# rrwick/Badread

Hardware: NVIDIA H100
Metric: simulated Gbases/sec (higher is better)
Workload: dtype u8/int32 (+f64 identity estimate)

## Files before the change

badread_b200/csrc/bb_api.cu:

```cuda
#include <cuda_runtime.h>
#include <dlfcn.h>
#include <unistd.h>

#include <algorithm>
#include <atomic>
#include <cstdio>
#include <cstdlib>
#include <cstring>
#include <numeric>
#include <string>
#include <thread>
#include <vector>

#include "bb_kernels.cuh"
#include "bb_launch.h"

namespace {

struct DevBuf {
    void *p = nullptr;
    size_t cap = 0;
    bool borrowed = false;
    void borrow(const DevBuf &o) { release(); p = o.p; cap = o.cap; borrowed = true; }
    cudaError_t ensure(size_t bytes) {
// ... 59 lines not shown
    DevBuf d_red;
    cudaEvent_t ev_scan = nullptr;
    DevBuf d_read_index, d_seg_off, d_segs, d_lit, d_target, d_order, d_reads;
    int n_lane_reads = 0, n_long_reads = 0;
    std::vector<int> h_order;
    DevBuf d_kidx, d_frag, d_state, d_seq, d_ops, d_dcnt, d_qual, d_out_seq, d_out_qual, d_counter, d_fpeq, d_speq, d_fallback;
    int64_t fpeq_total = 0;

    int n_warps = 0;
    BBScratchPool pool{}, pool_lean{};
    DevBuf s_hist, s_hbuf, s_lr, s_stack, s_tbuf, s_peq, s_ltbuf, s_leafhist, s_lr_lean, s_wckpt, s_lanehist;
    DevBuf d_ctime, d_chlog, d_wres, d_wtasks, d_wfallback, d_active;
    DevBuf p_q, p_t, p_ops, p_dcnt, p_out, p_qual;
    int lane8_cols = 4096;
    int pair_ctas = 1;
    bool head_worker = true;
    bool is_head = false;
    bool lpt_order = true;
    int ring_t = 4;
    bool lowmem = false;
    bool use_quad = false;
    int grid_div_env = 0;
    int grid_div = 1;
    struct QueueBufs { DevBuf node[BBQ_NODE_CLASSES][2], leaf[2], count; } qbuf[2];


    cudaEvent_t ev[BB_N_STAGES + 1] = {};
    float stage_ms[BB_N_STAGES] = {};

    std::vector<bb_ctx *> kids;
    int n_split = 1;
    std::vector<std::vector<int32_t>> part;
    std::vector<int64_t> part_base;
    cudaEvent_t ev_t0 = nullptr, ev_t1 = nullptr;

    bool trace = false;
    struct Mark { const char *name; int stream; cudaEvent_t ev; };
    std::vector<Mark> marks;
    std::vector<cudaEvent_t> mark_pool;
    size_t mark_used = 0;
};

static void mark(bb_ctx *ctx, cudaStream_t st, const char *name) {
    if (!ctx->trace) return;
    if (ctx->mark_used == ctx->mark_pool.size()) {
        cudaEvent_t e;
        if (cudaEventCreate(&e) != cudaSuccess) return;
// ... 135 lines not shown
    cudaEventCreate(&ctx->ev_t1);
    return BB_OK;
}

extern "C" int bb_destroy(bb_ctx *ctx) {
    if (!ctx) return BB_OK;
    for (bb_ctx *kid : ctx->kids) bb_destroy(kid);
    ctx->kids.clear();
    cudaSetDevice(ctx->device);
    cudaStreamSynchronize(ctx->stream);
    if (ctx->ev_t0) cudaEventDestroy(ctx->ev_t0);
    if (ctx->ev_t1) cudaEventDestroy(ctx->ev_t1);
    DevBuf *bufs[] = {&ctx->ref, &ctx->em_k2r, &ctx->em_hentries, &ctx->em_rowoff, &ctx->em_cum, &ctx->em_flags, &ctx->em_slots,
                      &ctx->em_pool, &ctx->em_rowinfo, &ctx->qm_hkeys, &ctx->qm_hvals, &ctx->qm_lkeys, &ctx->qm_lpool, &ctx->qm_rowoff, &ctx->qm_scores, &ctx->qm_cum,
                      &ctx->d_read_index, &ctx->d_seg_off, &ctx->d_segs, &ctx->d_lit, &ctx->d_target, &ctx->d_order,
                      &ctx->d_reads, &ctx->d_kidx, &ctx->d_frag, &ctx->d_state, &ctx->d_seq, &ctx->d_ops, &ctx->d_dcnt,
                      &ctx->d_qual, &ctx->d_out_seq, &ctx->d_out_qual, &ctx->d_counter, &ctx->s_hist, &ctx->s_hbuf,
                      &ctx->s_lr, &ctx->s_stack, &ctx->s_tbuf, &ctx->s_peq, &ctx->s_ltbuf, &ctx->d_ctime, &ctx->d_chlog, &ctx->d_wres,
                      &ctx->d_wtasks, &ctx->d_wfallback, &ctx->d_active,
                      &ctx->d_fpeq, &ctx->d_speq, &ctx->d_fallback, &ctx->s_leafhist, &ctx->s_lr_lean, &ctx->s_wckpt, &ctx->s_lanehist, &ctx->d_scan, &ctx->d_red,
                      &ctx->p_q, &ctx->p_t, &ctx->p_ops, &ctx->p_dcnt, &ctx->p_out, &ctx->p_qual};
    for (auto &qb : ctx->qbuf) {
        for (auto &cl : qb.node) for (auto &d : cl) d.release();
        qb.leaf[0].release(); qb.leaf[1].release(); qb.count.release();
    }
    for (DevBuf *b : bufs) b->release();
    for (auto &ev : ctx->ev) if (ev) cudaEventDestroy(ev);
    cudaStreamDestroy(ctx->stream);
    if (ctx->stream2) cudaStreamDestroy(ctx->stream2);
    if (ctx->ev_fork) cudaEventDestroy(ctx->ev_fork);
    if (ctx->ev_join) cudaEventDestroy(ctx->ev_join);
    if (ctx->ev_scan) cudaEventDestroy(ctx->ev_scan);
    for (int p = 0; p < 2; p++) {
        if (ctx->ev_level[p]) cudaEventDestroy(ctx->ev_level[p]);
        for (int x = 0; x < 3; x++) {
            if (ctx->side[p][x]) cudaStreamDestroy(ctx->side[p][x]);
            if (ctx->ev_side[p][x]) cudaEventDestroy(ctx->ev_side[p][x]);
        }
    }
    if (ctx->h_info) cudaFreeHost(ctx->h_info);
    if (ctx->nccl_comm && nccl_destroy) nccl_destroy(ctx->nccl_comm);
    for (cudaEvent_t e : ctx->mark_pool) cudaEventDestroy(e);
    delete ctx;
    return BB_OK;
}

template <typename T>
// ... 235 lines not shown
    {
        const size_t lanes = (size_t)lane_ctas * 64;
        if (ctx->lowmem) BB_CUDA(ctx, ctx->s_leafhist.ensure(2 * lanes * BB_LEAF_MAX_TILES * BB_LEAF_CKPT_WORDS * sizeof(uint32_t)));
        else BB_CUDA(ctx, ctx->s_lanehist.ensure(2 * lanes * BB_LEAF_LANE_COLS * BB_LEAF_LW * sizeof(uint2)));
        BB_CUDA(ctx, ctx->s_ltbuf.ensure(2 * lanes * BB_WIN_MAX_COLS));
        if (ctx->lowmem) BB_CUDA(ctx, ctx->s_wckpt.ensure(2 * lanes * BB_WIN_MAX_TILES * BB_WIN_CKPT_WORDS(BB_WIN_LW) * sizeof(uint32_t)));
    }
    const int len_b = (int)std::min<double>((double)ctx->max_len * ctx->slack + 64.0, (double)(1 << 24));
    const int lr_floor = ctx->lr_cap > 0 ? ctx->lr_cap : 4096;
    int lr_need = lr_floor;
    for (int r = 0; r < n; r++) {
        const double len = (double)ctx->h_reads[(size_t)r].frag_len;
        const double worst = len * ctx->slack + 64.0;
        const double expect = ctx->lr_cap > 0 ? 0.0 : 3.0 * (1.0 - ctx->h_target[(size_t)r]) * len + 0.02 * len + 512.0;
        lr_need = std::max(lr_need, (int)std::min(worst, ctx->lr_worst ? worst : expect));
    }
    int rc = ensure_scratch(ctx, len_b, lr_need, len_b, lr_floor);
    if (rc) return rc;
    const int cap_node = (int)std::min<int64_t>(ctx->seq_cap / 256 + 4ll * n + 1024, 0x7ffffff0);
    for (int s = 0; s < 2; s++) {
        auto &qb = ctx->qbuf[s];
        for (int c = 0; c < BBQ_NODE_CLASSES; c++)
            for (int p = 0; p < 2; p++) BB_CUDA(ctx, qb.node[c][p].ensure((size_t)cap_node * sizeof(BBNode)));
        for (int w = 0; w < 2; w++) BB_CUDA(ctx, qb.leaf[w].ensure((size_t)cap_node * sizeof(BBNode)));
        BB_CUDA(ctx, qb.count.ensure(512 * sizeof(int)));
    }
    ctx->n_levels = std::max(1, std::min(48, level_bound(ctx->max_len, ctx->slack) + ctx->extra_levels));
    return BB_OK;
}

static int w_batch_upload(bb_ctx *ctx, int32_t n_reads, const uint64_t *read_index, const int32_t *seg_off,
                          const bb_segment *segs, const uint8_t *literal_pool, int64_t literal_len,
                          const double *target_identity) {
    if (!ctx) return BB_ERR_ARG;
    if (n_reads <= 0 || !read_index || !seg_off || !segs || !target_identity || literal_len < 0)
        return set_err(ctx, BB_ERR_ARG, "bb_batch_upload: bad arguments");
    if (!ctx->have_em || !ctx->have_qm) return set_err(ctx, BB_ERR_STATE, "upload the error and qscore models first");
    BB_CUDA(ctx, cudaSetDevice(ctx->device));
    const int k = ctx->em.k;
    ctx->h_reads.assign((size_t)n_reads, BBReadDev{});
    ctx->h_inlen.assign((size_t)n_reads, 0);
    ctx->h_target.assign(target_identity, target_identity + n_reads);
    int64_t off = 0, peq_off = 0, log_off = 0, wres_off = 0;
    int max_len = 0;
    for (int32_t r = 0; r < n_reads; r++) {
        int64_t len = 0;
        if (seg_off[r + 1] < seg_off[r]) return set_err(ctx, BB_ERR_ARG, "seg_off must be non-decreasing");
// ... 85 lines not shown
                                 ctx->s_lanehist.as<uint2>(), ctx->s_ltbuf.as<uint8_t>(), c + BBC_LANE8, fb2, c + BBC_FB2);
        mark(ctx, st, "window_lane8");
        bbl_window_warp(pgrid(ctx, 2), st, B, ctx->em, ctx->pool, fb2, c + BBC_FB2, ctx->seed, c + BBC_WARP);
        mark(ctx, st, "window_warp");
        bb_k_replay<<<(n + 3) / 4, 128, 0, st>>>(B, order, n, ctx->em.k, c + BBC_PENDING);
        mark(ctx, st, "replay");
        ctx->launches += 6;
    }
    return BB_OK;
}

static int enqueue_align_tasks(bb_ctx *ctx, const BBBatchDev &B) {
    cudaStream_t stream[2] = {ctx->stream, ctx->stream2};
    const int n = ctx->n_reads;
    const int cap_node = (int)std::min<int64_t>(ctx->seq_cap / 256 + 4ll * n + 1024, 0x7ffffff0);
    const int lane_ctas = ctx->sm_count * 4;
    const size_t hist_per_pipe = (size_t)lane_ctas * 64 * BB_LEAF_MAX_TILES * BB_LEAF_CKPT_WORDS;
    BBQueues Q[2];
    int *cnt[2];
    for (int s = 0; s < 2; s++) {
        auto &qb = ctx->qbuf[s];
        for (int c = 0; c < BBQ_NODE_CLASSES; c++)
            for (int p = 0; p < 2; p++) Q[s].node[c][p] = qb.node[c][p].as<BBNode>();
        for (int w = 0; w < 2; w++) Q[s].leaf[w] = qb.leaf[w].as<BBNode>();
        cnt[s] = qb.count.as<int>();
        Q[s].count = cnt[s]; Q[s].overflow = cnt[s] + BBQ_OVERFLOW; Q[s].cap_node = cap_node; Q[s].cap_leaf = cap_node;
        Q[s].lane8_cols = ctx->lane8_cols;
        BB_CUDA(ctx, cudaMemsetAsync(cnt[s], 0, 512 * sizeof(int), stream[0]));
    }
    bb_k_push_roots<<<(n + 255) / 256, 256, 0, stream[0]>>>(B, Q[0], Q[1], ctx->d_order.as<int>());
    ctx->launches++;
    BB_CUDA(ctx, cudaEventRecord(ctx->ev_fork, stream[0]));
    BB_CUDA(ctx, cudaStreamWaitEvent(stream[1], ctx->ev_fork, 0));
    int *cursor[2] = {cnt[0] + 16, cnt[1] + 16};
    const int warp_base[2] = {0, ctx->n_warps / 2};
    const int w4 = ctx->sm_count * 4 * BB_WARPS_PER_CTA, w2 = ctx->sm_count * 6 * BB_WARPS_PER_CTA;
    const int lean_base[2] = {0, w4 + 2 * w2};
    for (int level = 0; level < ctx->n_levels; level++) {
        const int p = (level & 1) | (level > 0 && ctx->lpt_order ? BBQ_BACKWARDS : 0);
        for (int s = 0; s < 2; s++) {
            cudaStream_t st = stream[s];
            BB_CUDA(ctx, cudaMemsetAsync(cnt[s] + BBQ_COUNT(0, (p & 1) ^ 1), 0, BBQ_NODE_CLASSES * sizeof(int), st));
            BB_CUDA(ctx, cudaEventRecord(ctx->ev_level[s], st));
            int n_side = 0;
            auto on_side = [&]() -> cudaStream_t {
                cudaStream_t x = ctx->side[s][n_side++];
                cudaStreamWaitEvent(x, ctx->ev_level[s], 0);
                mark(ctx, x, "fork");
                return x;
            };
// ... 7 lines not shown
            {
                cudaStream_t x = on_side();
                bbl_node_warp(2, std::min(pgrid(ctx, 3, "WARP2"), ctx->sm_count * 6), x, B, Q[s], ctx->pool_lean, p, cursor[s]++, lean_base[s] + w4);
                mark(ctx, x, "node_warp2");
                bbl_node_warp(1, std::min(pgrid(ctx, 3, "WARP1"), ctx->sm_count * 6), x, B, Q[s], ctx->pool_lean, p, cursor[s]++, lean_base[s] + w4 + w2);
                mark(ctx, x, "node_warp1");
                x = on_side();
                bbl_node_lane8(pgrid(ctx, 6, "LANE8"), x, B, Q[s], p, cursor[s]++);
                mark(ctx, x, "node_lane8");
            }
            bbl_node_warp(4, std::min(pgrid(ctx, 2, "WARP4"), ctx->sm_count * 4), st, B, Q[s], ctx->pool_lean, p, cursor[s]++, lean_base[s]);
            mark(ctx, st, "node_warp4");
            ctx->launches += 4;
            for (int x = 0; x < n_side; x++) {
                BB_CUDA(ctx, cudaEventRecord(ctx->ev_side[s][x], ctx->side[s][x]));
                BB_CUDA(ctx, cudaStreamWaitEvent(st, ctx->ev_side[s][x], 0));
            }
        }
    }
    for (int s = 0; s < 2; s++) {
        cudaStream_t st = stream[s];
        bbl_leaf_warp(ctx->sm_count, st, B, Q[s], ctx->pool, cursor[s]++, warp_base[s]);
        mark(ctx, st, "leaf_warp");
        if (ctx->lowmem)
            bbl_leaf_lane(std::min(pgrid(ctx, 3, "LEAF"), ctx->sm_count * 4), st, B, Q[s], ctx->s_leafhist.as<uint32_t>() + s * hist_per_pipe, cursor[s]++);
        else
            bbl_leaf_lane_hist(std::min(pgrid(ctx, 4, "LEAF"), ctx->sm_count * 4), st, B, Q[s],
                               ctx->s_lanehist.as<uint2>() + s * ((size_t)lane_ctas * 64 * BB_LEAF_LANE_COLS * BB_LEAF_LW), cursor[s]++);
        mark(ctx, st, "leaf_lane");
        ctx->launches += 2;
    }
    BB_CUDA(ctx, cudaEventRecord(ctx->ev_join, stream[1]));
    BB_CUDA(ctx, cudaStreamWaitEvent(stream[0], ctx->ev_join, 0));
    for (int s = 0; s < 2; s++)
        BB_CUDA(ctx, cudaMemcpyAsync(ctx->h_info->qcount[s], cnt[s], 32 * sizeof(int), cudaMemcpyDeviceToHost, stream[0]));
    return BB_OK;
}

static int w_enqueue(bb_ctx *ctx) {
    if (!ctx) return BB_ERR_ARG;
    if (!ctx->uploaded) return set_err(ctx, BB_ERR_STATE, "bb_batch_run: no batch uploaded");
    BB_CUDA(ctx, cudaSetDevice(ctx->device));
    cudaStream_t st = ctx->stream;
    const int n = ctx->n_reads;
    BBBatchDev B = batch_dev(ctx);
    ctx->finished = false;
    BB_CUDA(ctx, cudaMemcpyAsync(ctx->d_reads.p, ctx->h_reads.data(), (size_t)n * sizeof(BBReadDev), cudaMemcpyHostToDevice, st));
    BB_CUDA(ctx, cudaMemsetAsync(ctx->d_counter.p, 0, BB_N_COUNTERS * sizeof(int), st));
    ctx->marks.clear(); ctx->mark_used = 0;
    mark(ctx, st, "begin");
    BB_CUDA(ctx, cudaEventRecord(ctx->ev[0], st));
    if (ctx->em.type == 1 && ctx->em_hash.entries)
        bb_k_build_fragments<0, true><<<n, 256, 0, st>>>(B, ctx->ref.as<uint8_t>(), ctx->em.k, ctx->seed, nullptr, ctx->em_hash);
// ... 602 lines not shown
```

badread_b200/csrc/bb_lane.cuh:

```cuda
#pragma once
#include <cstdint>

#include "bb_align.cuh"

struct BBLaneProb {
    const uint4 *peq;
    int peq_bit0;
    const uint8_t *q;
    int n;
    const uint8_t *t;
    int m;
    int a, b;
    uint2 *hist;
};

__device__ __forceinline__ int bb_lane_words(int a, int b) { return ((a + b) >> 5) + 2; }

__device__ __forceinline__ void bb_lane_fetch(const BBLaneProb &P, int word, uint32_t &mA, uint32_t &mC, uint32_t &mG,
                                              uint32_t &mT) {
    mA = mC = mG = mT = 0u;
    const int R = word * 32;
    const int valid = P.n - R;
    if (valid <= 0) return;
    const int s = P.peq_bit0 + R;
// ... 113 lines not shown

#define BB_RING_BYTES(LW, T) (2 * (T) * (LW) * 64 * 8)

__device__ __forceinline__ void bb_cp_async8(uint2 *smem, const uint2 *gmem) {
#if defined(__CUDA_ARCH__)
    asm volatile("cp.async.ca.shared.global [%0], [%1], 8;" ::"r"((uint32_t)__cvta_generic_to_shared(smem)), "l"(gmem) : "memory");
#else
    *smem = *gmem;
#endif
}
__device__ __forceinline__ void bb_cp_async_commit() {
#if defined(__CUDA_ARCH__)
    asm volatile("cp.async.commit_group;" ::: "memory");
#endif
}
template <int N>
__device__ __forceinline__ void bb_cp_async_wait() {
#if defined(__CUDA_ARCH__)
    asm volatile("cp.async.wait_group %0;" ::"n"(N) : "memory");
#endif
}

template <int LW, int T>
__device__ __forceinline__ void bb_ring_tick(uint2 *ring, const uint2 *hist, int tj, int &staged_lo) {
    const bool fresh = staged_lo > tj;
    if (fresh) {
        const int lo1 = max(0, tj - T + 1);
        for (int col = tj; col >= lo1; col--) {
#pragma unroll
            for (int x = 0; x < LW; x++) bb_cp_async8(ring + ((col & (2 * T - 1)) * LW + x) * 64, hist + (long long)col * LW + x);
        }
        bb_cp_async_commit();
        staged_lo = lo1;
    }
    const int want_lo = max(0, tj - 2 * T + 1);
    for (int col = staged_lo - 1; col >= want_lo; col--) {
#pragma unroll
        for (int x = 0; x < LW; x++) bb_cp_async8(ring + ((col & (2 * T - 1)) * LW + x) * 64, hist + (long long)col * LW + x);
    }
    bb_cp_async_commit();
    if (want_lo < staged_lo) staged_lo = want_lo;
#if defined(__CUDA_ARCH__)
    {
        constexpr int LINES = (T * LW * 8 + 127) / 128 + 1;
        const long long e = ((long long)tj - 4 * T) * LW;
#pragma unroll
        for (int x = 0; x < 2 * LINES; x++)
            if (e + 16 * x >= 0 && (x < LINES || fresh)) asm volatile("prefetch.global.L2 [%0];" ::"l"(hist + e + 16 * x));
    }
#endif
    bb_cp_async_wait<1>();
}

template <int LW, int T>
__device__ __forceinline__ uint2 bb_ring_entry(const uint2 *ring, int col, int x) {
    return ring[((col & (2 * T - 1)) * LW + x) * 64];
}
```

badread_b200/csrc/bb_launch.h:

```cpp
#pragma once
#include <cuda_runtime.h>

#include "bb_kernels.cuh"

void bbl_mutate(int grid, cudaStream_t st, BBBatchDev B, BBErrorModelDev em, unsigned long long seed, int *work_counter,
                const int *order, int n_items, bool chain);
cudaError_t bbl_window_lane_init();
void bbl_window_lane4(int grid, cudaStream_t st, BBBatchDev B, BBErrorModelDev em, const BBWinTask *tasks, const int *n_tasks,
                      unsigned long long seed, uint32_t *ckpt_pool, uint8_t *tbuf_pool, int *cursor, BBWinTask *fallback,
                      int *fallback_count);
void bbl_window_lane8(int grid, cudaStream_t st, BBBatchDev B, BBErrorModelDev em, const BBWinTask *tasks, const int *n_tasks,
                      unsigned long long seed, uint32_t *ckpt_pool, uint8_t *tbuf_pool, int *cursor, BBWinTask *fallback,
                      int *fallback_count);
void bbl_window_lane_hist(int words, int ring_t, int grid, cudaStream_t st, BBBatchDev B, BBErrorModelDev em, const BBWinTask *tasks,
                          const int *n_tasks, unsigned long long seed, uint2 *hist_pool, uint8_t *tbuf_pool, int *cursor,
                          BBWinTask *fallback, int *fallback_count);
void bbl_window_warp(int grid, cudaStream_t st, BBBatchDev B, BBErrorModelDev em, BBScratchPool pool, const BBWinTask *tasks,
                     const int *n_tasks, unsigned long long seed, int *cursor);
void bbl_node_warp(int words, int grid, cudaStream_t st, BBBatchDev B, BBQueues Q, BBScratchPool pool, int parity, int *cursor,
                   int warp_base);
void bbl_node_lane8(int grid, cudaStream_t st, BBBatchDev B, BBQueues Q, int parity, int *cursor);
cudaError_t bbl_node_quad_init();
void bbl_node_quad(int grid, cudaStream_t st, BBBatchDev B, BBQueues Q, BBScratchPool pool, int parity, int *cursor,
                   int warp_base);
cudaError_t bbl_node_pair_init();
void bbl_node_pair(int grid, cudaStream_t st, BBBatchDev B, BBQueues Q, BBScratchPool pool, int parity, int *cursor,
                   int warp_base);
void bbl_leaf_warp(int grid, cudaStream_t st, BBBatchDev B, BBQueues Q, BBScratchPool pool, int *cursor, int warp_base);
void bbl_leaf_lane_hist(int grid, cudaStream_t st, BBBatchDev B, BBQueues Q, uint2 *hist_pool, int *cursor);
cudaError_t bbl_leaf_lane_init();
void bbl_leaf_lane(int grid, cudaStream_t st, BBBatchDev B, BBQueues Q, uint32_t *ckpt_pool, int *cursor);
void bbl_align_pair(cudaStream_t st, const uint8_t *q, int n, const uint8_t *t, int m, int k_upper, BBScratchPool pool,
                    uint8_t *ops, unsigned int *dcnt, int *out5);
```

badread_b200/csrc/bb_loop.cuh:

```cuda
#pragma once
#include <cstdint>

#include "bb_lane.cuh"

enum { BB_STOP_HORIZON = 0, BB_STOP_LIMIT = 1, BB_STOP_COUNT = 2, BB_STOP_NOLOOP = 3 };

#define BB_WIN_LW 8
#define BB_WIN_MAX_COLS 2048

struct BBWinTask { int r, a; };

#define BB_MUTP_THREADS (BB_WARPS_PER_CTA * 32 + 32)

template <int BB_TU_ = 0>
__global__ void __launch_bounds__(BB_MUTP_THREADS)
bb_k_mutate(BBBatchDev B, BBErrorModelDev em, unsigned long long seed, int *work_counter, const int *order,
                 int n_items) {
    constexpr int NE = BB_WARPS_PER_CTA * 32;
    __shared__ int s_kind[2][NE], s_pos[2][NE], s_rpos[2][NE];
    __shared__ uint32_t s_pay[2][NE];
    __shared__ int s_w, s_stop, s_cc;
    __shared__ long long s_n0;
    const int lane = threadIdx.x & 31;
    const int warp = threadIdx.x >> 5;
// ... 414 lines not shown
#endif
template <int LW, int T = BB_WIN_RING_T>
__global__ void __launch_bounds__(64, (LW <= 4 ? 8 : 4))
bb_k_window_lane_hist(BBBatchDev B, BBErrorModelDev em, const BBWinTask *tasks, const int *n_tasks_ptr, unsigned long long seed,
                 uint2 *hist_pool, uint8_t *tbuf_pool, int *cursor, BBWinTask *fallback, int *fallback_count) {
#ifdef BB_EMULATOR
    static uint2 s_ring[BB_RING_BYTES(LW, T) / 8];
#else
    extern __shared__ __align__(16) uint2 s_ring[];
#endif
    const int n_tasks = *n_tasks_ptr;
    const long long gl = (long long)blockIdx.x * blockDim.x + threadIdx.x;
    uint2 *const hist = hist_pool + gl * (long long)(BB_WIN_MAX_COLS * LW);
    uint8_t *const tbuf = tbuf_pool + gl * (long long)BB_WIN_MAX_COLS;
    uint2 *const ring = s_ring + threadIdx.x;
    BBLanePass<LW> S;
    BBProb P;
    BBWinTask tk = {0, 0};
    const uint8_t *frag = nullptr;
    const uint32_t *state = nullptr;
    const unsigned int *ctime = nullptr;
    int phase = 0;
    int qpos = 0, qn = 0, jx = 0, tm = 0, uw = 0, ti = 0, tj = 0, diags = 0, dels = 0, dist = 0, staged_lo = 0;
    unsigned int tmax = 0;
    for (;;) {
        if (phase == 0) {
            const int w = atomicAdd(cursor, 1);
            if (w >= n_tasks) phase = 4;
            else {
                tk = tasks[w];
                const BBReadDev *rd = &B.reads[tk.r];
                frag = B.frag + rd->frag_off; state = B.state + rd->frag_off; ctime = B.ctime + rd->frag_off;
                bb_window_of(rd->frag_len, seed, B.read_index[tk.r], tk.a, qpos, qn);
                tmax = (unsigned int)(BB_ALIGNMENT_INTERVAL * tk.a);
                jx = 0; tm = 0; uw = 0;
                phase = 1;
            }
        }
        if (__all_sync(BB_FULL, phase == 4)) break;
        for (int it = 0; it < 64; it++) {
            if (phase == 1) {
                unsigned int ct4[4];
                uint8_t fb4[4];
#pragma unroll
                for (int h = 0; h < 4; h++) {
                    const int j = min(jx + h, qn - 1);
// ... 6 lines not shown
                        if (ct4[h] == 0u || ct4[h] > tmax) { if (tm < BB_WIN_MAX_COLS) tbuf[tm] = fb4[h]; tm++; }
                        else {
                            const uint32_t st = state[qpos + jx];
                            const int sl = (int)(st & 0xff);
                            for (int c = 0; c < sl; c++) { if (tm < BB_WIN_MAX_COLS) tbuf[tm] = bb_slot_char(em, st, c); tm++; }
                            uw += sl < 1 ? 1 : sl;
                        }
                        jx++;
                    }
                }
                if (jx >= qn) {
                    const int diff = qn > tm ? qn - tm : tm - qn;
                    if (uw < diff) uw = diff;
                    const int mx = qn > tm ? qn : tm;
                    if (uw > mx) uw = mx;
                    bb_band(qn, tm, uw, P.a, P.b);
                    if (tm > BB_WIN_MAX_COLS || bb_lane_words(P.a, P.b) > LW || !bb_uses_traceback(qn, tm)) {
                        fallback[atomicAdd(fallback_count, 1)] = tk;
                        phase = 0;
                    } else {
                        const BBReadDev *rd = &B.reads[tk.r];
                        P.n = qn; P.peq = B.fpeq + rd->fpeq_off; P.q = frag + qpos; P.qs = 1;
                        P.peq_bit0 = qpos + BB_PEQ_BIT0; P.t = tbuf; P.ts = 1;
                        bb_lane_begin<LW>(S, P);
                        phase = 2;
                    }
                }
            }
        }
        for (int it = 0; it < 128; it++) {
            if (phase == 2) {
                bb_lane_step<LW, true>(S, P, hist + (long long)S.c * LW);
                if (S.c >= tm) {
                    dist = bb_lane_corner<LW>(S, qn);
                    ti = qn - 1; tj = tm - 1; diags = 0; dels = 0; staged_lo = tm; phase = 3;
                }
            }
        }
        for (int it = 0; it < 256; it++) {
            if (phase == 3) {
                if (ti >= 0 && tj >= 0) {
                    if ((it & (T - 1)) == 0) bb_ring_tick<LW, T>(ring, hist, tj, staged_lo);
                    int wt = (tj - P.a) >> 5; if (wt < 0) wt = 0;
                    const int x = (ti >> 5) - wt;
                    if (x < 0 || x >= LW) { atomicOr(&B.reads[tk.r].flags, 1); ti = -1; tj = -1; }
                    else {
                        const uint2 e = bb_ring_entry<LW, T>(ring, tj, x);
                        const int bit = ti & 31;
                        if ((e.x >> bit) & 1u) ti--;
                        else if ((e.y >> bit) & 1u) { dels++; tj--; }
                        else { diags++; ti--; tj--; }
                    }
                } else {
                    bb_cp_async_wait<0>();
                    if (tj >= 0) dels += tj + 1;
                    const int matches = diags - (dist - (qn - diags) - dels);
                    if (dist >= BB_INF) atomicOr(&B.reads[tk.r].flags, 1);
                    B.wres[B.reads[tk.r].wres_off + tk.a - 1] = make_int2(matches, qn + dels);
                    phase = 0;
                }
            }
        }
    }
}

template <int BB_TU_ = 0>
__global__ void __launch_bounds__(BB_WARPS_PER_CTA * 32, 4)
bb_k_window_warp(BBBatchDev B, BBErrorModelDev em, BBScratchPool pool, const BBWinTask *tasks, const int *n_tasks_ptr,
// ... 150 lines not shown
```

badread_b200/csrc/bb_tasks.cuh:

```cuda
#pragma once
#include <cstdint>

#include "bb_align.cuh"
#include "bb_lane.cuh"

#define BB_NODE_LW_SMALL 8
#define BB_LEAF_LW 8
#define BB_LEAF_LANE_COLS 2048

enum { BBQ_NODE_LANE8 = 0, BBQ_NODE_LEAN1 = 1, BBQ_NODE_LEAN2 = 2, BBQ_NODE_LEAN4 = 3, BBQ_NODE_WIDE = 4, BBQ_NODE_CLASSES = 5 };
#define BBQ_COUNT(cls, parity) ((parity) * BBQ_NODE_CLASSES + (cls))
#define BBQ_LEAF_COUNT 10
#define BBQ_OVERFLOW 12
#define BBQ_BACKWARDS 2

struct BBNode { int r, q0, nn, t0, mm, best; };

struct BBQueues {
    BBNode *node[BBQ_NODE_CLASSES][2];
    BBNode *leaf[2];
    int *count;
    int *overflow;
    int cap_node, cap_leaf;
    int lane8_cols;
};

struct BBAlignOut {
    uint8_t *ops;
    unsigned int *dcnt;
    BBReadDev *rd;
};

__device__ __forceinline__ void bb_add_dels(const BBAlignOut &o, int qidx_after, int count) {
    if (count <= 0) return;
    if (qidx_after >= 0) atomicAdd(&o.dcnt[qidx_after], (unsigned int)count);
    else atomicAdd(&o.rd->lead_del, count);
}

__device__ __forceinline__ void bb_task_band(const BBNode &nd, int upper, int &a, int &b) {
    int k = nd.best >= 0 ? nd.best : upper;
    const int diff = nd.nn > nd.mm ? nd.nn - nd.mm : nd.mm - nd.nn;
    if (k < diff) k = diff;
    const int mx = nd.nn > nd.mm ? nd.nn : nd.mm;
    if (k > mx) k = mx;
    bb_band(nd.nn, nd.mm, k, a, b);
    a += a & 1; b += b & 1;
}

static __device__ void bb_push_task(const BBQueues &Q, int next_parity, const BBAlignOut &o, const BBNode &nd, int upper) {
    if (nd.nn == 0) {
        atomicAdd(&o.rd->dels, nd.mm);
        bb_add_dels(o, nd.q0 - 1, nd.mm);
        return;
    }
    if (nd.mm == 0) {
        for (int x = 0; x < nd.nn; x++) o.ops[nd.q0 + x] = BB_OP_I;
        return;
    }
    int a, b;
    bb_task_band(nd, upper, a, b);
    const int lw = bb_lane_words(a, b);
    if (bb_uses_traceback(nd.nn, nd.mm)) {
        const int which = (lw <= BB_LEAF_LW && nd.mm <= BB_LEAF_LANE_COLS) ? 0 : 1;
        const int idx = atomicAdd(&Q.count[BBQ_LEAF_COUNT + which], 1);
        if (idx >= Q.cap_leaf) { atomicExch(Q.overflow, 1); return; }
        Q.leaf[which][idx] = nd;
    } else {
        const int L2 = bb_pick_L<4>(a, b, 16);
        const int cls = (lw <= BB_NODE_LW_SMALL && nd.mm <= Q.lane8_cols) ? BBQ_NODE_LANE8
                        : L2 == 1 ? BBQ_NODE_LEAN1 : L2 == 2 ? BBQ_NODE_LEAN2 : L2 == 4 ? BBQ_NODE_LEAN4 : BBQ_NODE_WIDE;
        const int idx = atomicAdd(&Q.count[BBQ_COUNT(cls, next_parity)], 1);
        if (idx >= Q.cap_node) { atomicExch(Q.overflow, 1); return; }
        Q.node[cls][next_parity][idx] = nd;
    }
}

static __device__ bool bb_choose_split_seq(const int *L, int loL, int hiL, const int *R, int loR, int hiR, int nn, int left_w,
                                    int right_w, int &best, int &split, int &ls, int &rs) {
    int rlo = max(loL, nn - 2 - hiR); if (rlo < 0) rlo = 0;
    int rhi = min(hiL, nn - 2 - loR); if (rhi > nn - 2) rhi = nn - 2;
    const bool have_top = nn - 1 >= loR && nn - 1 <= hiR;
    const bool have_bot = nn - 1 >= loL && nn - 1 <= hiL;
    if (best < 0) {
        int mn = BB_INF;
        for (int r = rlo; r <= rhi; r++) mn = min(mn, L[r - loL] + R[(nn - 2 - r) - loR]);
        if (have_top) mn = min(mn, left_w + R[(nn - 1) - loR]);
// ... 28 lines not shown
    int a, b;
    bb_task_band(nd, rd->upper, a, b);
    const bool wide = !bb_uses_traceback(nd.nn, nd.mm) && bb_pick_L<4>(a, b, 16) == 0;
    bb_push_task(wide ? QW : QN, 0, o, nd, rd->upper);
}

template <int LW>
struct BBLanePass {
    uint32_t Pv[LW], Mv[LW], eA[LW], eC[LW], eG[LW], eT[LW];
    int wt, score, c;
};

template <int LW>
__device__ __forceinline__ void bb_lane_begin(BBLanePass<LW> &S, const BBProb &P) {
#pragma unroll
    for (int x = 0; x < LW; x++) {
        S.Pv[x] = ~0u; S.Mv[x] = 0u;
        bb_fetch_peq(P, 32 * x, S.eA[x], S.eC[x], S.eG[x], S.eT[x]);
    }
    S.wt = 0; S.score = 32 * LW; S.c = 0;
}

template <int LW, bool HIST, int HSTRIDE = 1>
__device__ __forceinline__ void bb_lane_step(BBLanePass<LW> &S, const BBProb &P, uint2 *hist) {
    const int c = S.c;
    if (c - P.a >= 32 * (S.wt + 1)) {
#pragma unroll
        for (int x = 0; x + 1 < LW; x++) {
            S.Pv[x] = S.Pv[x + 1]; S.Mv[x] = S.Mv[x + 1];
            S.eA[x] = S.eA[x + 1]; S.eC[x] = S.eC[x + 1]; S.eG[x] = S.eG[x + 1]; S.eT[x] = S.eT[x + 1];
        }
        S.wt++;
        S.Pv[LW - 1] = ~0u; S.Mv[LW - 1] = 0u;
        bb_fetch_peq(P, 32 * (S.wt + LW - 1), S.eA[LW - 1], S.eC[LW - 1], S.eG[LW - 1], S.eT[LW - 1]);
        S.score += 32;
    }
    const uint32_t tc = P.t[(long long)c * P.ts];
    const uint32_t code = (tc >> 1) & 3u;
    const bool acgt = ((0x47544341u >> (8 * code)) & 0xffu) == tc;
    uint32_t Eq[LW], Xv[LW], A[LW], Sm[LW], Ph[LW], Mh[LW];
#pragma unroll
    for (int x = 0; x < LW; x++)
        Eq[x] = (code & 2u) ? ((code & 1u) ? S.eG[x] : S.eT[x]) : ((code & 1u) ? S.eC[x] : S.eA[x]);
    if (!acgt) {
#pragma unroll
        for (int x = 0; x < LW; x++) {
            Eq[x] = 0u;
            const int row0 = (S.wt + x) * 32;
            for (int r = 0; r < 32; r++)
                if (row0 + r < P.n && P.q[(long long)(row0 + r) * P.qs] == tc) Eq[x] |= 1u << r;
        }
    }
#pragma unroll
    for (int x = 0; x < LW; x++) { Xv[x] = Eq[x] | S.Mv[x]; A[x] = Eq[x] & S.Pv[x]; }
    bb_add_words<LW>(A, S.Pv, Sm);
#pragma unroll
    for (int x = 0; x < LW; x++) {
        const uint32_t Xh = (Sm[x] ^ S.Pv[x]) | Eq[x];
        Ph[x] = S.Mv[x] | ~(Xh | S.Pv[x]);
        Mh[x] = S.Pv[x] & Xh;
    }
    S.score += (int)(Ph[LW - 1] >> 31) - (int)(Mh[LW - 1] >> 31);
#pragma unroll
    for (int x = LW - 1; x >= 0; x--) {
        const uint32_t phs = __funnelshift_l(x > 0 ? Ph[x - 1] : 0x80000000u, Ph[x], 1);
        const uint32_t mhs = __funnelshift_l(x > 0 ? Mh[x - 1] : 0u, Mh[x], 1);
        const uint32_t raw = Ph[x];
        S.Pv[x] = mhs | ~(Xv[x] | phs);
        S.Mv[x] = phs & Xv[x];
        if (HIST && (HSTRIDE != 1 || (LW & 1))) hist[x * HSTRIDE] = make_uint2(S.Pv[x], raw);
        if (HIST && HSTRIDE == 1 && !(LW & 1)) Ph[x] = raw;
    }
    if (HIST && HSTRIDE == 1 && !(LW & 1)) {
#pragma unroll
        for (int x = 0; x < LW; x += 2)
            reinterpret_cast<uint4 *>(hist)[x >> 1] = make_uint4(S.Pv[x], Ph[x], S.Pv[x + 1], Ph[x + 1]);
    }
    S.c = c + 1;
}

template <int LW>
__device__ int bb_lane_column_scores(const BBLanePass<LW> &S, int n, int lo, int hi, int *out) {
    int result = BB_INF;
    int run = S.score;
#pragma unroll
    for (int x = LW - 1; x >= 0; x--) {
        const int row0 = (S.wt + x) * 32;
        int rr = run;
        for (int r = 31; r >= 0; r--) {
            const int row = row0 + r;
            if (row < n) {
                if (out && row >= lo && row <= hi) out[row - lo] = rr;
                if (row == n - 1) result = rr;
            }
            rr -= (int)((S.Pv[x] >> r) & 1u) - (int)((S.Mv[x] >> r) & 1u);
        }
        run -= __popc(S.Pv[x]) - __popc(S.Mv[x]);
    }
    return result;
// ... 176 lines not shown
                            o.ops[nd.q0 + ti] = eq ? BB_OP_EQ : BB_OP_X;
                            matches += eq ? 1 : 0;
                            ti--; tj--;
                        }
                    }
                    if (ti < 0 || tj < 0) walking = false;
                    else if (tj < tile_lo) need_tile = true;
                }
            }
        }
        if (active) {
            if (walking) atomicOr(&o.rd->flags, 1 << 8);
            for (int x = 0; x <= ti; x++) o.ops[nd.q0 + x] = BB_OP_I;
            if (tj >= 0) { bb_add_dels(o, nd.q0 - 1, tj + 1); dels += tj + 1; }
            atomicAdd(&o.rd->matches, matches);
            atomicAdd(&o.rd->dels, dels);
        }
    }
}

#ifndef BB_LEAF_RING_T
#define BB_LEAF_RING_T 4
#endif
#define BB_LEAF_RING_BYTES BB_RING_BYTES(BB_LEAF_LW, BB_LEAF_RING_T)

template <int BB_TU_ = 0>
__global__ void __launch_bounds__(64)
bb_k_leaf_lane_hist(BBBatchDev B, BBQueues Q, uint2 *hist_pool, int *cursor) {
    constexpr int LW = BB_LEAF_LW, T = BB_LEAF_RING_T;
#ifdef BB_EMULATOR
    static uint2 s_ring[BB_LEAF_RING_BYTES / 8];
#else
    extern __shared__ __align__(16) uint2 s_ring[];
#endif
    const BBNode *list = Q.leaf[0];
    const int count = min(Q.count[BBQ_LEAF_COUNT], Q.cap_leaf);
    uint2 *const hist = hist_pool + ((long long)blockIdx.x * blockDim.x + threadIdx.x) * (long long)(BB_LEAF_LANE_COLS * LW);
    uint2 *const ring = s_ring + threadIdx.x;
    BBLanePass<LW> S;
    BBProb P;
    BBNode nd;
    BBAlignOut o;
    const uint8_t *qp = nullptr, *tp = nullptr;
    int phase = 0;
    int ti = 0, tj = 0, matches = 0, dels = 0, staged_lo = 0;
    for (;;) {
        if (phase == 0) {
            const int w = atomicAdd(cursor, 1);
            if (w >= count) phase = 3;
            else {
                nd = list[w];
                BBReadDev *rd = &B.reads[nd.r];
                o.ops = B.ops + rd->seq_off; o.dcnt = B.dcnt + rd->seq_off; o.rd = rd;
                bb_task_band(nd, rd->upper, P.a, P.b);
                P.n = nd.nn; P.peq = B.speq + rd->speq_off;
                qp = B.seq + rd->seq_off + nd.q0; tp = B.frag + rd->frag_off + nd.t0;
                P.q = qp; P.qs = 1; P.peq_bit0 = nd.q0 + BB_PEQ_BIT0; P.t = tp; P.ts = 1;
                bb_lane_begin<LW>(S, P);
                phase = 1;
            }
        }
        if (__all_sync(BB_FULL, phase == 3)) break;
        for (int it = 0; it < 128; it++) {
            if (phase == 1) {
                bb_lane_step<LW, true>(S, P, hist + (long long)S.c * LW);
                if (S.c >= nd.mm) {
                    const int d = bb_lane_corner<LW>(S, nd.nn);
                    if (nd.best >= 0 && d != nd.best) atomicOr(&o.rd->flags, 8 << 8);
                    ti = nd.nn - 1; tj = nd.mm - 1; matches = 0; dels = 0; staged_lo = nd.mm;
                    phase = 2;
                }
            }
        }
        for (int it = 0; it < 256; it++) {
            if (phase == 2) {
                if (ti >= 0 && tj >= 0) {
                    if ((it & (T - 1)) == 0) bb_ring_tick<LW, T>(ring, hist, tj, staged_lo);
                    int wt = (tj - P.a) >> 5; if (wt < 0) wt = 0;
                    const int x = (ti >> 5) - wt;
                    if (x < 0 || x >= LW) { atomicOr(&o.rd->flags, 1 << 8); ti = -1; tj = -1; }
                    else {
                        const uint2 e = bb_ring_entry<LW, T>(ring, tj, x);
                        const int bit = ti & 31;
                        if ((e.x >> bit) & 1u) { o.ops[nd.q0 + ti] = BB_OP_I; ti--; }
                        else if ((e.y >> bit) & 1u) { bb_add_dels(o, nd.q0 + ti, 1); dels++; tj--; }
                        else {
                            const bool eq = qp[ti] == tp[tj];
                            o.ops[nd.q0 + ti] = eq ? BB_OP_EQ : BB_OP_X;
                            matches += eq ? 1 : 0;
                            ti--; tj--;
                        }
                    }
                } else {
                    bb_cp_async_wait<0>();
                    for (int x = 0; x <= ti; x++) o.ops[nd.q0 + x] = BB_OP_I;
                    if (tj >= 0) { bb_add_dels(o, nd.q0 - 1, tj + 1); dels += tj + 1; }
                    atomicAdd(&o.rd->matches, matches);
                    atomicAdd(&o.rd->dels, dels);
                    phase = 0;
                }
            }
        }
    }
// ... 275 lines not shown
```

badread_b200/csrc/bb_tu_leaf.cu:

```cuda
#include "bb_launch.h"

void bbl_leaf_warp(int grid, cudaStream_t st, BBBatchDev B, BBQueues Q, BBScratchPool pool, int *cursor, int warp_base) {
    bb_k_leaf_warp<<<grid, BB_WARPS_PER_CTA * 32, 0, st>>>(B, Q, pool, cursor, warp_base);
}

cudaError_t bbl_leaf_lane_init() {
    return cudaFuncSetAttribute(bb_k_leaf_lane<0>, cudaFuncAttributeMaxDynamicSharedMemorySize, BB_LEAF_SMEM_BYTES);
}

void bbl_leaf_lane(int grid, cudaStream_t st, BBBatchDev B, BBQueues Q, uint32_t *ckpt_pool, int *cursor) {
    bb_k_leaf_lane<0><<<grid, 64, BB_LEAF_SMEM_BYTES, st>>>(B, Q, ckpt_pool, cursor);
}

void bbl_leaf_lane_hist(int grid, cudaStream_t st, BBBatchDev B, BBQueues Q, uint2 *hist_pool, int *cursor) {
    bb_k_leaf_lane_hist<0><<<grid, 64, BB_LEAF_RING_BYTES, st>>>(B, Q, hist_pool, cursor);
}
```

Before: 1.098.

## Route narrow-band leaf tasks to a dedicated 4-word lane kernel with compact history

```diff
diff --git a/badread_b200/csrc/bb_api.cu b/badread_b200/csrc/bb_api.cu
--- a/badread_b200/csrc/bb_api.cu
+++ b/badread_b200/csrc/bb_api.cu
@@ -105,7 +105,7 @@
     bool use_quad = false;
     int grid_div_env = 0;
     int grid_div = 1;
-    struct QueueBufs { DevBuf node[BBQ_NODE_CLASSES][2], leaf[2], count; } qbuf[2];
+    struct QueueBufs { DevBuf node[BBQ_NODE_CLASSES][2], leaf[3], count; } qbuf[2];
 
 
     cudaEvent_t ev[BB_N_STAGES + 1] = {};
@@ -287,7 +287,8 @@
                       &ctx->p_q, &ctx->p_t, &ctx->p_ops, &ctx->p_dcnt, &ctx->p_out, &ctx->p_qual};
     for (auto &qb : ctx->qbuf) {
         for (auto &cl : qb.node) for (auto &d : cl) d.release();
-        qb.leaf[0].release(); qb.leaf[1].release(); qb.count.release();
+        for (auto &d : qb.leaf) d.release();
+        qb.count.release();
     }
     for (DevBuf *b : bufs) b->release();
     for (auto &ev : ctx->ev) if (ev) cudaEventDestroy(ev);
@@ -569,7 +570,7 @@
         auto &qb = ctx->qbuf[s];
         for (int c = 0; c < BBQ_NODE_CLASSES; c++)
             for (int p = 0; p < 2; p++) BB_CUDA(ctx, qb.node[c][p].ensure((size_t)cap_node * sizeof(BBNode)));
-        for (int w = 0; w < 2; w++) BB_CUDA(ctx, qb.leaf[w].ensure((size_t)cap_node * sizeof(BBNode)));
+        for (auto &d : qb.leaf) BB_CUDA(ctx, d.ensure((size_t)cap_node * sizeof(BBNode)));
         BB_CUDA(ctx, qb.count.ensure(512 * sizeof(int)));
     }
     ctx->n_levels = std::max(1, std::min(48, level_bound(ctx->max_len, ctx->slack) + ctx->extra_levels));
@@ -701,10 +702,11 @@
         auto &qb = ctx->qbuf[s];
         for (int c = 0; c < BBQ_NODE_CLASSES; c++)
             for (int p = 0; p < 2; p++) Q[s].node[c][p] = qb.node[c][p].as<BBNode>();
-        for (int w = 0; w < 2; w++) Q[s].leaf[w] = qb.leaf[w].as<BBNode>();
+        for (int w = 0; w < 3; w++) Q[s].leaf[w] = qb.leaf[w].as<BBNode>();
         cnt[s] = qb.count.as<int>();
         Q[s].count = cnt[s]; Q[s].overflow = cnt[s] + BBQ_OVERFLOW; Q[s].cap_node = cap_node; Q[s].cap_leaf = cap_node;
         Q[s].lane8_cols = ctx->lane8_cols;
+        Q[s].leaf_lane4 = ctx->lowmem ? 0 : 1;
         BB_CUDA(ctx, cudaMemsetAsync(cnt[s], 0, 512 * sizeof(int), stream[0]));
     }
     bb_k_push_roots<<<(n + 255) / 256, 256, 0, stream[0]>>>(B, Q[0], Q[1], ctx->d_order.as<int>());
@@ -758,13 +760,18 @@
         cudaStream_t st = stream[s];
         bbl_leaf_warp(ctx->sm_count, st, B, Q[s], ctx->pool, cursor[s]++, warp_base[s]);
         mark(ctx, st, "leaf_warp");
-        if (ctx->lowmem)
+        ctx->launches++;
+        if (ctx->lowmem) {
             bbl_leaf_lane(std::min(pgrid(ctx, 3, "LEAF"), ctx->sm_count * 4), st, B, Q[s], ctx->s_leafhist.as<uint32_t>() + s * hist_per_pipe, cursor[s]++);
-        else
-            bbl_leaf_lane_hist(std::min(pgrid(ctx, 4, "LEAF"), ctx->sm_count * 4), st, B, Q[s],
-                               ctx->s_lanehist.as<uint2>() + s * ((size_t)lane_ctas * 64 * BB_LEAF_LANE_COLS * BB_LEAF_LW), cursor[s]++);
+            ctx->launches++;
+        } else {
+            uint2 *pool = ctx->s_lanehist.as<uint2>() + s * ((size_t)lane_ctas * 64 * BB_LEAF_LANE_COLS * BB_LEAF_LW);
+            bbl_leaf_lane_hist(4, std::min(pgrid(ctx, 8, "LEAF4"), ctx->sm_count * 8), st, B, Q[s], pool, cursor[s]++);
+            mark(ctx, st, "leaf_lane4");
+            bbl_leaf_lane_hist(BB_LEAF_LW, std::min(pgrid(ctx, 4, "LEAF"), ctx->sm_count * 4), st, B, Q[s], pool, cursor[s]++);
+            ctx->launches += 2;
+        }
         mark(ctx, st, "leaf_lane");
-        ctx->launches += 2;
     }
     BB_CUDA(ctx, cudaEventRecord(ctx->ev_join, stream[1]));
     BB_CUDA(ctx, cudaStreamWaitEvent(stream[0], ctx->ev_join, 0));
diff --git a/badread_b200/csrc/bb_lane.cuh b/badread_b200/csrc/bb_lane.cuh
--- a/badread_b200/csrc/bb_lane.cuh
+++ b/badread_b200/csrc/bb_lane.cuh
@@ -159,13 +159,14 @@
 }
 
 template <int LW, int T>
-__device__ __forceinline__ void bb_ring_tick(uint2 *ring, const uint2 *hist, int tj, int &staged_lo) {
+__device__ __forceinline__ void bb_ring_tick(uint2 *ring, const uint2 *hist, int hw, int tj, int &staged_lo) {
     const bool fresh = staged_lo > tj;
     if (fresh) {
         const int lo1 = max(0, tj - T + 1);
         for (int col = tj; col >= lo1; col--) {
 #pragma unroll
-            for (int x = 0; x < LW; x++) bb_cp_async8(ring + ((col & (2 * T - 1)) * LW + x) * 64, hist + (long long)col * LW + x);
+            for (int x = 0; x < LW; x++)
+                if (x < hw) bb_cp_async8(ring + ((col & (2 * T - 1)) * LW + x) * 64, hist + (long long)col * hw + x);
         }
         bb_cp_async_commit();
         staged_lo = lo1;
@@ -173,17 +174,20 @@
     const int want_lo = max(0, tj - 2 * T + 1);
     for (int col = staged_lo - 1; col >= want_lo; col--) {
 #pragma unroll
-        for (int x = 0; x < LW; x++) bb_cp_async8(ring + ((col & (2 * T - 1)) * LW + x) * 64, hist + (long long)col * LW + x);
+        for (int x = 0; x < LW; x++)
+            if (x < hw) bb_cp_async8(ring + ((col & (2 * T - 1)) * LW + x) * 64, hist + (long long)col * hw + x);
     }
     bb_cp_async_commit();
     if (want_lo < staged_lo) staged_lo = want_lo;
 #if defined(__CUDA_ARCH__)
     {
-        constexpr int LINES = (T * LW * 8 + 127) / 128 + 1;
-        const long long e = ((long long)tj - 4 * T) * LW;
+        constexpr int MAX_LINES = (T * LW * 8 + 127) / 128 + 1;
+        const int lines = (T * hw * 8 + 127) / 128 + 1;
+        const long long e = ((long long)tj - 4 * T) * hw;
 #pragma unroll
-        for (int x = 0; x < 2 * LINES; x++)
-            if (e + 16 * x >= 0 && (x < LINES || fresh)) asm volatile("prefetch.global.L2 [%0];" ::"l"(hist + e + 16 * x));
+        for (int x = 0; x < 2 * MAX_LINES; x++)
+            if (e + 16 * x >= 0 && (x < lines || (fresh && x < 2 * lines)))
+                asm volatile("prefetch.global.L2 [%0];" ::"l"(hist + e + 16 * x));
     }
 #endif
     bb_cp_async_wait<1>();
diff --git a/badread_b200/csrc/bb_launch.h b/badread_b200/csrc/bb_launch.h
--- a/badread_b200/csrc/bb_launch.h
+++ b/badread_b200/csrc/bb_launch.h
@@ -27,7 +27,8 @@
 void bbl_node_pair(int grid, cudaStream_t st, BBBatchDev B, BBQueues Q, BBScratchPool pool, int parity, int *cursor,
                    int warp_base);
 void bbl_leaf_warp(int grid, cudaStream_t st, BBBatchDev B, BBQueues Q, BBScratchPool pool, int *cursor, int warp_base);
-void bbl_leaf_lane_hist(int grid, cudaStream_t st, BBBatchDev B, BBQueues Q, uint2 *hist_pool, int *cursor);
+void bbl_leaf_lane_hist(int words, int grid, cudaStream_t st, BBBatchDev B, BBQueues Q, uint2 *hist_pool,
+                        int *cursor);
 cudaError_t bbl_leaf_lane_init();
 void bbl_leaf_lane(int grid, cudaStream_t st, BBBatchDev B, BBQueues Q, uint32_t *ckpt_pool, int *cursor);
 void bbl_align_pair(cudaStream_t st, const uint8_t *q, int n, const uint8_t *t, int m, int k_upper, BBScratchPool pool,
diff --git a/badread_b200/csrc/bb_loop.cuh b/badread_b200/csrc/bb_loop.cuh
--- a/badread_b200/csrc/bb_loop.cuh
+++ b/badread_b200/csrc/bb_loop.cuh
@@ -460,6 +460,7 @@
     const unsigned int *ctime = nullptr;
     int phase = 0;
     int qpos = 0, qn = 0, jx = 0, tm = 0, uw = 0, ti = 0, tj = 0, diags = 0, dels = 0, dist = 0, staged_lo = 0;
+    int hw = LW;
     unsigned int tmax = 0;
     for (;;) {
         if (phase == 0) {
@@ -512,6 +513,7 @@
                         const BBReadDev *rd = &B.reads[tk.r];
                         P.n = qn; P.peq = B.fpeq + rd->fpeq_off; P.q = frag + qpos; P.qs = 1;
                         P.peq_bit0 = qpos + BB_PEQ_BIT0; P.t = tbuf; P.ts = 1;
+                        hw = bb_lane_words(P.a, P.b);
                         bb_lane_begin<LW>(S, P);
                         phase = 2;
                     }
@@ -520,7 +522,7 @@
         }
         for (int it = 0; it < 128; it++) {
             if (phase == 2) {
-                bb_lane_step<LW, true>(S, P, hist + (long long)S.c * LW);
+                bb_lane_step<LW, true>(S, P, hist + (long long)S.c * hw, hw);
                 if (S.c >= tm) {
                     dist = bb_lane_corner<LW>(S, qn);
                     ti = qn - 1; tj = tm - 1; diags = 0; dels = 0; staged_lo = tm; phase = 3;
@@ -530,10 +532,10 @@
         for (int it = 0; it < 256; it++) {
             if (phase == 3) {
                 if (ti >= 0 && tj >= 0) {
-                    if ((it & (T - 1)) == 0) bb_ring_tick<LW, T>(ring, hist, tj, staged_lo);
+                    if ((it & (T - 1)) == 0) bb_ring_tick<LW, T>(ring, hist, hw, tj, staged_lo);
                     int wt = (tj - P.a) >> 5; if (wt < 0) wt = 0;
                     const int x = (ti >> 5) - wt;
-                    if (x < 0 || x >= LW) { atomicOr(&B.reads[tk.r].flags, 1); ti = -1; tj = -1; }
+                    if (x < 0 || x >= hw) { atomicOr(&B.reads[tk.r].flags, 1); ti = -1; tj = -1; }
                     else {
                         const uint2 e = bb_ring_entry<LW, T>(ring, tj, x);
                         const int bit = ti & 31;
diff --git a/badread_b200/csrc/bb_tasks.cuh b/badread_b200/csrc/bb_tasks.cuh
--- a/badread_b200/csrc/bb_tasks.cuh
+++ b/badread_b200/csrc/bb_tasks.cuh
@@ -10,19 +10,21 @@
 
 enum { BBQ_NODE_LANE8 = 0, BBQ_NODE_LEAN1 = 1, BBQ_NODE_LEAN2 = 2, BBQ_NODE_LEAN4 = 3, BBQ_NODE_WIDE = 4, BBQ_NODE_CLASSES = 5 };
 #define BBQ_COUNT(cls, parity) ((parity) * BBQ_NODE_CLASSES + (cls))
+enum { BBQ_LEAF_LANE = 0, BBQ_LEAF_WARP = 1, BBQ_LEAF_LANE4 = 2 };
 #define BBQ_LEAF_COUNT 10
-#define BBQ_OVERFLOW 12
+#define BBQ_OVERFLOW 13
 #define BBQ_BACKWARDS 2
 
 struct BBNode { int r, q0, nn, t0, mm, best; };
 
 struct BBQueues {
     BBNode *node[BBQ_NODE_CLASSES][2];
-    BBNode *leaf[2];
+    BBNode *leaf[3] = {};
     int *count;
     int *overflow;
     int cap_node, cap_leaf;
     int lane8_cols;
+    int leaf_lane4 = 0;
 };
 
 struct BBAlignOut {
@@ -61,7 +63,8 @@
     bb_task_band(nd, upper, a, b);
     const int lw = bb_lane_words(a, b);
     if (bb_uses_traceback(nd.nn, nd.mm)) {
-        const int which = (lw <= BB_LEAF_LW && nd.mm <= BB_LEAF_LANE_COLS) ? 0 : 1;
+        const int which = nd.mm > BB_LEAF_LANE_COLS || lw > BB_LEAF_LW ? BBQ_LEAF_WARP
+                          : lw <= 4 && Q.leaf_lane4 ? BBQ_LEAF_LANE4 : BBQ_LEAF_LANE;
         const int idx = atomicAdd(&Q.count[BBQ_LEAF_COUNT + which], 1);
         if (idx >= Q.cap_leaf) { atomicExch(Q.overflow, 1); return; }
         Q.leaf[which][idx] = nd;
@@ -136,7 +139,7 @@
 }
 
 template <int LW, bool HIST, int HSTRIDE = 1>
-__device__ __forceinline__ void bb_lane_step(BBLanePass<LW> &S, const BBProb &P, uint2 *hist) {
+__device__ __forceinline__ void bb_lane_step(BBLanePass<LW> &S, const BBProb &P, uint2 *hist, int hw = LW) {
     const int c = S.c;
     if (c - P.a >= 32 * (S.wt + 1)) {
 #pragma unroll
@@ -182,13 +185,18 @@
         const uint32_t raw = Ph[x];
         S.Pv[x] = mhs | ~(Xv[x] | phs);
         S.Mv[x] = phs & Xv[x];
-        if (HIST && (HSTRIDE != 1 || (LW & 1))) hist[x * HSTRIDE] = make_uint2(S.Pv[x], raw);
-        if (HIST && HSTRIDE == 1 && !(LW & 1)) Ph[x] = raw;
-    }
-    if (HIST && HSTRIDE == 1 && !(LW & 1)) {
-#pragma unroll
-        for (int x = 0; x < LW; x += 2)
-            reinterpret_cast<uint4 *>(hist)[x >> 1] = make_uint4(S.Pv[x], Ph[x], S.Pv[x + 1], Ph[x + 1]);
+        if (HIST && HSTRIDE != 1) hist[x * HSTRIDE] = make_uint2(S.Pv[x], raw);
+    }
+    if (HIST && HSTRIDE == 1) {
+        if (!(hw & 1)) {
+#pragma unroll
+            for (int x = 0; x + 1 < LW; x += 2)
+                if (x < hw) reinterpret_cast<uint4 *>(hist)[x >> 1] = make_uint4(S.Pv[x], Ph[x], S.Pv[x + 1], Ph[x + 1]);
+        } else {
+#pragma unroll
+            for (int x = 0; x < LW; x++)
+                if (x < hw) hist[x] = make_uint2(S.Pv[x], Ph[x]);
+        }
     }
     S.c = c + 1;
 }
@@ -411,19 +419,21 @@
 #ifndef BB_LEAF_RING_T
 #define BB_LEAF_RING_T 4
 #endif
-#define BB_LEAF_RING_BYTES BB_RING_BYTES(BB_LEAF_LW, BB_LEAF_RING_T)
-
-template <int BB_TU_ = 0>
-__global__ void __launch_bounds__(64)
+#define BB_LEAF_RING_BYTES_LW(LW) BB_RING_BYTES(LW, BB_LEAF_RING_T)
+#define BB_LEAF_RING_BYTES BB_LEAF_RING_BYTES_LW(BB_LEAF_LW)
+
+template <int LW = BB_LEAF_LW>
+__global__ void __launch_bounds__(64, (LW <= 4 ? 8 : 1))
 bb_k_leaf_lane_hist(BBBatchDev B, BBQueues Q, uint2 *hist_pool, int *cursor) {
-    constexpr int LW = BB_LEAF_LW, T = BB_LEAF_RING_T;
+    constexpr int T = BB_LEAF_RING_T;
+    constexpr int QUEUE = LW <= 4 ? BBQ_LEAF_LANE4 : BBQ_LEAF_LANE;
 #ifdef BB_EMULATOR
-    static uint2 s_ring[BB_LEAF_RING_BYTES / 8];
+    static uint2 s_ring[BB_LEAF_RING_BYTES_LW(LW) / 8];
 #else
     extern __shared__ __align__(16) uint2 s_ring[];
 #endif
-    const BBNode *list = Q.leaf[0];
-    const int count = min(Q.count[BBQ_LEAF_COUNT], Q.cap_leaf);
+    const BBNode *list = Q.leaf[QUEUE];
+    const int count = min(Q.count[BBQ_LEAF_COUNT + QUEUE], Q.cap_leaf);
     uint2 *const hist = hist_pool + ((long long)blockIdx.x * blockDim.x + threadIdx.x) * (long long)(BB_LEAF_LANE_COLS * LW);
     uint2 *const ring = s_ring + threadIdx.x;
     BBLanePass<LW> S;
@@ -432,7 +442,7 @@
     BBAlignOut o;
     const uint8_t *qp = nullptr, *tp = nullptr;
     int phase = 0;
-    int ti = 0, tj = 0, matches = 0, dels = 0, staged_lo = 0;
+    int ti = 0, tj = 0, matches = 0, dels = 0, staged_lo = 0, hw = LW;
     for (;;) {
         if (phase == 0) {
             const int w = atomicAdd(cursor, 1);
@@ -445,6 +455,7 @@
                 P.n = nd.nn; P.peq = B.speq + rd->speq_off;
                 qp = B.seq + rd->seq_off + nd.q0; tp = B.frag + rd->frag_off + nd.t0;
                 P.q = qp; P.qs = 1; P.peq_bit0 = nd.q0 + BB_PEQ_BIT0; P.t = tp; P.ts = 1;
+                hw = bb_lane_words(P.a, P.b);
                 bb_lane_begin<LW>(S, P);
                 phase = 1;
             }
@@ -452,7 +463,7 @@
         if (__all_sync(BB_FULL, phase == 3)) break;
         for (int it = 0; it < 128; it++) {
             if (phase == 1) {
-                bb_lane_step<LW, true>(S, P, hist + (long long)S.c * LW);
+                bb_lane_step<LW, true>(S, P, hist + (long long)S.c * hw, hw);
                 if (S.c >= nd.mm) {
                     const int d = bb_lane_corner<LW>(S, nd.nn);
                     if (nd.best >= 0 && d != nd.best) atomicOr(&o.rd->flags, 8 << 8);
@@ -464,10 +475,10 @@
         for (int it = 0; it < 256; it++) {
             if (phase == 2) {
                 if (ti >= 0 && tj >= 0) {
-                    if ((it & (T - 1)) == 0) bb_ring_tick<LW, T>(ring, hist, tj, staged_lo);
+                    if ((it & (T - 1)) == 0) bb_ring_tick<LW, T>(ring, hist, hw, tj, staged_lo);
                     int wt = (tj - P.a) >> 5; if (wt < 0) wt = 0;
                     const int x = (ti >> 5) - wt;
-                    if (x < 0 || x >= LW) { atomicOr(&o.rd->flags, 1 << 8); ti = -1; tj = -1; }
+                    if (x < 0 || x >= hw) { atomicOr(&o.rd->flags, 1 << 8); ti = -1; tj = -1; }
                     else {
                         const uint2 e = bb_ring_entry<LW, T>(ring, tj, x);
                         const int bit = ti & 31;
diff --git a/badread_b200/csrc/bb_tu_leaf.cu b/badread_b200/csrc/bb_tu_leaf.cu
--- a/badread_b200/csrc/bb_tu_leaf.cu
+++ b/badread_b200/csrc/bb_tu_leaf.cu
@@ -12,6 +12,7 @@
     bb_k_leaf_lane<0><<<grid, 64, BB_LEAF_SMEM_BYTES, st>>>(B, Q, ckpt_pool, cursor);
 }
 
-void bbl_leaf_lane_hist(int grid, cudaStream_t st, BBBatchDev B, BBQueues Q, uint2 *hist_pool, int *cursor) {
-    bb_k_leaf_lane_hist<0><<<grid, 64, BB_LEAF_RING_BYTES, st>>>(B, Q, hist_pool, cursor);
+void bbl_leaf_lane_hist(int words, int grid, cudaStream_t st, BBBatchDev B, BBQueues Q, uint2 *hist_pool, int *cursor) {
+    if (words == 4) bb_k_leaf_lane_hist<4><<<grid, 64, BB_LEAF_RING_BYTES_LW(4), st>>>(B, Q, hist_pool, cursor);
+    else bb_k_leaf_lane_hist<BB_LEAF_LW><<<grid, 64, BB_LEAF_RING_BYTES, st>>>(B, Q, hist_pool, cursor);
 }
```

New measurement: 1.130, median of 6. 1.03x the previous value.
